# kuldeepbrd1/graspLDM

Measured on AMD Instinct MI355X. Metric: grasps/sec whole-node (1024-pt cloud, 100 DDIM steps), higher is better.
Workload: dtype f32 (GEMMs as split-f16 x3 partial products on the f16 matrix pipe, f32 accumulation; GroupNorm / LayerNorm / attention / scheduler in f32); 1 GPU; LDM mode, 256 synthetic 1024-pt clouds per GPU x 20 grasps, 100 DDIM steps: BASELINE.json configs[2] per GPU (configs[3] = this per-GPU workload on 8 GPUs); experiment=fpc, clouds_per_gpu=256, grasps_per_cloud=20, points=1024, ddim_steps=100, encoder=PVCNNEncoder (shipped fpc config), parallelism=cloud-sharded x1, weights=synthetic recipe seed 0, streams=3

## Files before the change

### graspldm_amd/csrc/quad_narrow.h

```cpp
#ifndef GLDM_QUAD_NARROW_H_
#define GLDM_QUAD_NARROW_H_

#ifdef GLDM_DEBUG_KNOBS
__device__ long long g_q_stamp[4][16];
#define GLDM_QSTAMP(c, i) do { if (blockIdx.x == 0 && (c).lane == 0) g_q_stamp[(c).wave & 3][i] = (long long)__builtin_readcyclecounter(); } while (0)
#else
#define GLDM_QSTAMP(c, i) do {} while (0)
#endif

template <int CTRL>
__device__ __forceinline__ float dpp_zero(float x) {
  return __int_as_float(__builtin_amdgcn_update_dpp(0, __float_as_int(x), CTRL, 0xf, 0xf, true));
}
template <int CTRL>
__device__ __forceinline__ u32x4 dpp_zero4(const u32x4 &v) {
  u32x4 o;
#pragma unroll
  for (int i = 0; i < 4; ++i) o[i] = (unsigned)__builtin_amdgcn_update_dpp(0, (int)v[i], CTRL, 0xf, 0xf, true);
  return o;
}
__device__ __forceinline__ float pos_sum(float v) {
  v += dpp_mov<0x124>(v);
  return v + dpp_mov<0x128>(v);
}
__device__ __forceinline__ float pos_max(float v) { return dpp_max<0x128>(dpp_max<0x124>(v)); }
#define GLDM_DPP8_STAGE1(op, i, j) "v_" op "_f32_dpp %" #i ", %" #j ", %" #j " row_ror:4 row_mask:0xf bank_mask:0xf\n\t"
#define GLDM_DPP8_STAGE2(op, i) "v_" op "_f32_dpp %" #i ", %" #i ", %" #i " row_ror:8 row_mask:0xf bank_mask:0xf\n\t"
#define GLDM_DPP8(op)                                                                                                  \
  "s_nop 1\n\t"                                                                                                         \
  GLDM_DPP8_STAGE1(op, 0, 8) GLDM_DPP8_STAGE1(op, 1, 9) GLDM_DPP8_STAGE1(op, 2, 10) GLDM_DPP8_STAGE1(op, 3, 11)          \
  GLDM_DPP8_STAGE1(op, 4, 12) GLDM_DPP8_STAGE1(op, 5, 13) GLDM_DPP8_STAGE1(op, 6, 14) GLDM_DPP8_STAGE1(op, 7, 15)        \
  GLDM_DPP8_STAGE2(op, 0) GLDM_DPP8_STAGE2(op, 1) GLDM_DPP8_STAGE2(op, 2) GLDM_DPP8_STAGE2(op, 3)                        \
  GLDM_DPP8_STAGE2(op, 4) GLDM_DPP8_STAGE2(op, 5) GLDM_DPP8_STAGE2(op, 6) GLDM_DPP8_STAGE2(op, 7)
#define GLDM_DPP8_OPERANDS                                                                                             \
  : "=&v"(r[0]), "=&v"(r[1]), "=&v"(r[2]), "=&v"(r[3]), "=&v"(r[4]), "=&v"(r[5]), "=&v"(r[6]), "=&v"(r[7])            \
  : "v"(x[0]), "v"(x[1]), "v"(x[2]), "v"(x[3]), "v"(x[4]), "v"(x[5]), "v"(x[6]), "v"(x[7])
#define GLDM_DPP8_STAGE1I(op, i) "v_" op "_f32_dpp %" #i ", %" #i ", %" #i " row_ror:4 row_mask:0xf bank_mask:0xf\n\t"
__device__ __forceinline__ void pos_max8(float (&x)[8]) {
  asm("s_nop 1\n\t"
      GLDM_DPP8_STAGE1I("max", 0) GLDM_DPP8_STAGE1I("max", 1) GLDM_DPP8_STAGE1I("max", 2) GLDM_DPP8_STAGE1I("max", 3)
      GLDM_DPP8_STAGE1I("max", 4) GLDM_DPP8_STAGE1I("max", 5) GLDM_DPP8_STAGE1I("max", 6) GLDM_DPP8_STAGE1I("max", 7)
      GLDM_DPP8_STAGE2("max", 0) GLDM_DPP8_STAGE2("max", 1) GLDM_DPP8_STAGE2("max", 2) GLDM_DPP8_STAGE2("max", 3)
      GLDM_DPP8_STAGE2("max", 4) GLDM_DPP8_STAGE2("max", 5) GLDM_DPP8_STAGE2("max", 6) GLDM_DPP8_STAGE2("max", 7)
      : "+v"(x[0]), "+v"(x[1]), "+v"(x[2]), "+v"(x[3]), "+v"(x[4]), "+v"(x[5]), "+v"(x[6]), "+v"(x[7]));
}
__device__ __forceinline__ void pos_sum8(const float (&x)[8], float (&r)[8]) {
  asm(GLDM_DPP8("add") GLDM_DPP8_OPERANDS);
}
__device__ __forceinline__ float kq_sum(float v) { return half_sum(row_pair_sum(v)); }
__device__ __forceinline__ float kq_max(float v) { return half_max(row_pair_max(v)); }

__device__ __forceinline__ void qsplit8(const f32x4 &a, const f32x4 &b, u32x4 (&pl)[kSplit]) {
  unsigned h, l;
  split_f16x2(a[0], a[1], h, l); pl[0][0] = h; pl[1][0] = l;
  split_f16x2(a[2], a[3], h, l); pl[0][1] = h; pl[1][1] = l;
  split_f16x2(b[0], b[1], h, l); pl[0][2] = h; pl[1][2] = l;
  split_f16x2(b[2], b[3], h, l); pl[0][3] = h; pl[1][3] = l;
}

enum { QM_OUT0 = 0, QM_SS2, QM_C1_2, QM_C2_2, QM_SS3, QM_C1_3, QM_C2_3, QM_QKV1, QM_OUT1, QM_DOWN1,
       QM_SS4, QM_C1_4, QM_C2_4, QM_SS5, QM_C1_5, QM_C2_5, QM_QKV2, QM_OUT2, QM_DOWN2, QM_COUNT };
struct QOff { int mat, a, b; };
constexpr QOff qconv_frag(int mat, int MT, int KB, int i, int mt0 = 0) {
  const int st = i / MT, mi = i % MT, kb = st / 3, t = st % 3;
  const int f = (mt0 + mi) * 3 * KB + t * KB + kb;
  return QOff{mat, 2048 * f, 2048 * f + 1024};
}
constexpr QOff qrb_frag(int mss, int MT, int KB, int i) {
  if (i < MT) return QOff{mss, 1024 * i, 1024 * (MT + i)};
  i -= MT;
  if (i < 3 * KB * MT) return qconv_frag(mss + 1, MT, KB, i);
  return qconv_frag(mss + 2, MT, KB, i - 3 * KB * MT);
}
constexpr int qrb_len(int MT, int KB) { return MT + 6 * KB * MT; }
constexpr QOff qatt_frag(int mqkv, int MT, int KB, int i) {
  const int per = 6 * KB + MT, h = i / per, r = i % per;
  if (r < 6 * KB) {
    const int mt6 = r / KB, kb = r % KB, part = mt6 / 2, half = mt6 % 2;
    const int f = (2 * h + half + 8 * part) * KB + kb;
    return QOff{mqkv, 2048 * f, 2048 * f + 1024};
  }
  const int f = (r - 6 * KB) * 4 + h;
  return QOff{mqkv + 1, 2048 * f, 2048 * f + 1024};
}
constexpr int qatt_len(int MT, int KB) { return 4 * (6 * KB + MT); }
constexpr int qlevel_len(int MT, int KB) { return 2 * qrb_len(MT, KB) + qatt_len(MT, KB) + 2 * MT * 3 * KB; }
constexpr QOff qlevel_frag(int m0, int MT, int KB, int DP, int i) {
  if (i < qrb_len(MT, KB)) return qrb_frag(m0, MT, KB, i);
  i -= qrb_len(MT, KB);
  if (i < qrb_len(MT, KB)) return qrb_frag(m0 + 3, MT, KB, i);
  i -= qrb_len(MT, KB);
  if (i < qatt_len(MT, KB)) return qatt_frag(m0 + 6, MT, KB, i);
  i -= qatt_len(MT, KB);
  const int pass = i / (DP * 3 * KB);
  return qconv_frag(m0 + 8, DP, KB, i % (DP * 3 * KB), DP * pass);
}
constexpr int kQN0 = 0;
constexpr int kQN1 = 4;
constexpr int kQN2 = kQN1 + qlevel_len(2, 1);
constexpr int kQNEnd = kQN2 + qlevel_len(4, 2);
constexpr QOff qstream_off(int n) {
  if (n < kQN1) return QOff{QM_OUT0, 2048 * n, 2048 * n + 1024};
  if (n < kQN2) return qlevel_frag(QM_SS2, 2, 1, 4, n - kQN1);
  return qlevel_frag(QM_SS4, 4, 2, 4, n - kQN2);
}

constexpr int kQG = 4;
constexpr int kQS = 32;
constexpr int kQGroups = kQNEnd / kQG;
static_assert(kQNEnd % kQG == 0 && kQS % kQG == 0, "whole groups");
constexpr int kQR = 6;
constexpr int kQSpinMax = 1 << 20;
__host__ __device__ constexpr int qslot_floats(int s) { return (s < 16 ? PG<4>::kH : PG<4>::kX + 4 * PG<4>::kBlockFloats) + (s & 15) * 512; }
static_assert(PG<4>::kH + 16 * 512 <= PG<4>::kX && PG<4>::kX + 4 * PG<4>::kBlockFloats + 16 * 512 <= 512 * 64, "slot regions");
typedef __attribute__((address_space(3))) int lds_i;
struct QStream4 {
  static constexpr int kEnd = kQNEnd, kGroups = kQGroups;
  static constexpr QOff off(int n) { return qstream_off(n); }
  __host__ __device__ static constexpr int slot_floats(int s) { return qslot_floats(s); }
};

struct QRing {
  u32x4 s[kQR][2];
  float *lds;
  lds_i *sync;
  int lane, quad;
  int flag;
  int spins = 0;
};
__device__ __forceinline__ int lds_poll(const lds_i *p) {
  int v;
  asm volatile("ds_read_b32 %0, %1\n\ts_waitcnt lgkmcnt(0)" : "=v"(v) : "v"(p) : "memory");
  return __builtin_amdgcn_readfirstlane(v);
}
template <int N, class ST = QStream4>
__device__ __forceinline__ void qring_load(QRing &ring) {
  if constexpr (N < ST::kEnd) {
    if constexpr (N % kQG == 0) {
      constexpr int g = N / kQG;
#if defined(GLDM_DEBUG_KNOBS) && defined(GLDM_QEXP_DUP)
      if (false) {
#else
      if (__builtin_expect(ring.flag != g + 1, 0)) {
#endif
        for (int spin = 0; spin < kQSpinMax && lds_poll(ring.sync + (g & 7)) != g + 1; ++spin) {
          __builtin_amdgcn_s_sleep(1);
#ifdef GLDM_DEBUG_KNOBS
          ++ring.spins;
#endif
        }
      }
      if constexpr (g + 1 < ST::kGroups) ring.flag = *(volatile lds_i *)(ring.sync + ((g + 1) & 7));
    }
#if defined(GLDM_DEBUG_KNOBS) && defined(GLDM_QEXP_NOLOAD)
    if (N >= kQR) return;
#endif
    const lds_u4 *slot = (const lds_u4 *)(ring.lds + ST::slot_floats(N % kQS)) + ring.lane;
    ring.s[N % kQR][0] = slot[0];
    ring.s[N % kQR][1] = slot[64];
  }
}
template <int N, class ST = QStream4>
__device__ __forceinline__ f32x4 qring_mfma(QRing &ring, const u32x4 (&b)[kSplit], f32x4 acc) {
#if defined(GLDM_DEBUG_KNOBS) && defined(GLDM_QEXP_NOMFMA)
  acc[0] += __uint_as_float(ring.s[N % kQR][0][0] ^ b[0][0]);
#else
  acc = mfma_split(ring.s[N % kQR], b, acc);
#endif
  if constexpr (N % kQG == kQG - 1) ring.sync[16 + 64 * ring.quad + ring.lane] = N / kQG + 1;
  if constexpr (N >= 1) qring_load<N - 1 + kQR, ST>(ring);
  return acc;
}

typedef __attribute__((address_space(3))) void lds_void;
typedef __attribute__((address_space(1))) const void glob_void;
__device__ __forceinline__ void quad_build_table(const gldm_r1d_desc &d, int *qtab, int tid, int nthreads) {
  const int mbf[QM_COUNT] = {d.lv[0].out_wq,
                             d.rb[2].ss_w, d.rb[2].c1_wq, d.rb[2].c2_wq, d.rb[3].ss_w, d.rb[3].c1_wq, d.rb[3].c2_wq,
                             d.lv[1].qkvn_wq, d.lv[1].out_wq, d.lv[1].down_wq,
                             d.rb[4].ss_w, d.rb[4].c1_wq, d.rb[4].c2_wq, d.rb[5].ss_w, d.rb[5].c1_wq, d.rb[5].c2_wq,
                             d.lv[2].qkvn_wq, d.lv[2].out_wq, d.lv[2].down_wq};
  for (int n = tid; n < kQNEnd; n += nthreads) {
    const QOff o = qstream_off(n);
    int base = 0;
#pragma unroll
    for (int m = 0; m < QM_COUNT; ++m) base = o.mat == m ? mbf[m] * 4 : base;
    qtab[2 * n] = base + o.a;
    qtab[2 * n + 1] = base + o.b;
  }
}
template <class ST = QStream4>
__device__ __forceinline__ void quad_loader(const Ctx &c) {
  using GG = Geo<64>;
  lds_i *sync = (lds_i *)(c.lds + GG::kMiscQ);
  const lds_i *qtab = (const lds_i *)(c.lds + GG::kMiscQTab);
  const char *wb = reinterpret_cast<const char *>(c.w) + c.lane * 16;
  for (int g = c.wave - 4; g < ST::kGroups; g += 4) {
    if (g >= 8) {
      for (int spin = 0; spin < kQSpinMax; ++spin) {
        const int d0 = lds_poll(sync + 16), d1 = lds_poll(sync + 80), d2 = lds_poll(sync + 144), d3 = lds_poll(sync + 208);
        if (min(min(d0, d1), min(d2, d3)) >= g - 7) break;
        __builtin_amdgcn_s_sleep(2);
      }
    }
    const int s0 = (g & 7) * kQG;
#pragma unroll
    for (int f = 0; f < kQG; ++f) {
      const int n = g * kQG + f;
      const int oa = __builtin_amdgcn_readfirstlane(qtab[2 * n]), ob = __builtin_amdgcn_readfirstlane(qtab[2 * n + 1]);
      const int sl = s0 + f;
      float *slot = c.lds + ST::slot_floats(sl);
      __builtin_amdgcn_global_load_lds((glob_void *)(wb + oa), (lds_void *)slot, 16, 0, 0);
      __builtin_amdgcn_global_load_lds((glob_void *)(wb + ob), (lds_void *)(slot + 256), 16, 0, 0);
    }
    asm volatile("s_waitcnt vmcnt(0)" ::: "memory");
    if (c.lane == 0) sync[g & 7] = g + 1;
  }
}

template <int N0, int MT, int KB, int SH = 4, class ST = QStream4>
__device__ __forceinline__ void qconv3(QRing &ring, const u32x4 (&xp)[KB][kSplit], f32x4 (&acc)[MT]) {
  using std::integral_constant;
  auto body = [&](auto st_c) {
    constexpr int st = decltype(st_c)::value, kb = st / 3, t = st % 3;
    u32x4 bs[kSplit];
#pragma unroll
    for (int pl = 0; pl < kSplit; ++pl)
      bs[pl] = t == 1 ? xp[kb][pl] : (t == 0 ? dpp_zero4<0x110 + SH>(xp[kb][pl]) : dpp_zero4<0x100 + SH>(xp[kb][pl]));
    auto per_m = [&](auto mi_c) {
      constexpr int mi = decltype(mi_c)::value;
      acc[mi] = qring_mfma<N0 + st * MT + mi, ST>(ring, bs, acc[mi]);
    };
    per_m(integral_constant<int, 0>{});
    if constexpr (MT > 1) per_m(integral_constant<int, 1>{});
    if constexpr (MT > 2) { per_m(integral_constant<int, 2>{}); per_m(integral_constant<int, 3>{}); }
    __builtin_amdgcn_sched_barrier(0);
  };
  body(integral_constant<int, 0>{}); body(integral_constant<int, 1>{}); body(integral_constant<int, 2>{});
  if constexpr (KB > 1) { body(integral_constant<int, 3>{}); body(integral_constant<int, 4>{}); body(integral_constant<int, 5>{}); }
}

template <int MT, int CPG>
__device__ __forceinline__ void qgn_stats(const f32x4 (&acc)[MT], float (&mean)[MT], float (&var)[MT]) {
  static_assert(CPG == 8 || CPG == 16, "groups of half an m-tile or a whole one");
  constexpr float inv_n = 1.0f / (float)(CPG * 4);
#pragma unroll
  for (int mi = 0; mi < MT; ++mi) {
    float s = (acc[mi][0] + acc[mi][1]) + (acc[mi][2] + acc[mi][3]);
    s = row_pair_sum(pos_sum(s));
    if (CPG == 16) s = half_sum(s);
    const float m = s * inv_n;
    float v = 0.f;
#pragma unroll
    for (int r = 0; r < 4; ++r) {
      const float d = acc[mi][r] - m;
      v = fmaf(d, d, v);
    }
    v = row_pair_sum(pos_sum(v));
    if (CPG == 16) v = half_sum(v);
    mean[mi] = m;
    var[mi] = v * inv_n;
  }
}

struct QRb { int c1_b, n1_w, n1_b, c2_b, n2_w, n2_b, ss_b; };

template <int N0, int MT, int KB>
__device__ __forceinline__ void quad_resblock(const Ctx &c, QRing &ring, const QRb &rb, f32x4 (&xr)[MT],
                                              u32x4 (&xp)[KB][kSplit], int smp) {
  using GG = Geo<64>;
  using std::integral_constant;
  constexpr int C = 16 * MT, CPG = C / 4;
  const int kq = c.lane >> 4;
  const float *w = c.w;
  const lds_f *Gs = (const lds_f *)(c.lds + GG::kMiscG) + smp * 16;
  float gb[4];
#pragma unroll
  for (int j = 0; j < 4; ++j) gb[j] = Gs[4 * j + kq];
  f32x4 sc[MT], sh[MT], g1[MT], be1[MT], b1[MT];
#pragma unroll
  for (int mi = 0; mi < MT; ++mi) {
    const int row0 = 16 * mi + 4 * kq;
    sc[mi] = *reinterpret_cast<const f32x4 *>(w + rb.ss_b + row0);
    sh[mi] = *reinterpret_cast<const f32x4 *>(w + rb.ss_b + C + row0);
    b1[mi] = *reinterpret_cast<const f32x4 *>(w + rb.c1_b + row0);
    g1[mi] = *reinterpret_cast<const f32x4 *>(w + rb.n1_w + row0);
    be1[mi] = *reinterpret_cast<const f32x4 *>(w + rb.n1_b + row0);
  }
  {
    auto ss_m = [&](auto mi_c) {
      constexpr int mi = decltype(mi_c)::value;
      const u32x4 a_sc = ring.s[(N0 + mi) % kQR][0], a_sh = ring.s[(N0 + mi) % kQR][1];
#pragma unroll
      for (int j = 0; j < 4; ++j) {
        sc[mi] = __builtin_amdgcn_mfma_f32_16x16x4f32(__uint_as_float(a_sc[j]), gb[j], sc[mi], 0, 0, 0);
        sh[mi] = __builtin_amdgcn_mfma_f32_16x16x4f32(__uint_as_float(a_sh[j]), gb[j], sh[mi], 0, 0, 0);
      }
      if constexpr (N0 + mi >= 1) qring_load<N0 + mi - 1 + kQR>(ring);
    };
    ss_m(integral_constant<int, 0>{}); ss_m(integral_constant<int, 1>{});
    if constexpr (MT > 2) { ss_m(integral_constant<int, 2>{}); ss_m(integral_constant<int, 3>{}); }
  }
  __builtin_amdgcn_sched_barrier(0);
  f32x4 acc[MT];
#pragma unroll
  for (int mi = 0; mi < MT; ++mi) acc[mi] = f32x4{0.f, 0.f, 0.f, 0.f};
  qconv3<N0 + MT, MT, KB>(ring, xp, acc);
  f32x4 b2[MT], g2[MT], be2[MT];
#pragma unroll
  for (int mi = 0; mi < MT; ++mi) {
    const int row0 = 16 * mi + 4 * kq;
    b2[mi] = *reinterpret_cast<const f32x4 *>(w + rb.c2_b + row0);
    g2[mi] = *reinterpret_cast<const f32x4 *>(w + rb.n2_w + row0);
    be2[mi] = *reinterpret_cast<const f32x4 *>(w + rb.n2_b + row0);
  }
#pragma unroll
  for (int mi = 0; mi < MT; ++mi)
#pragma unroll
    for (int r = 0; r < 4; ++r) acc[mi][r] += b1[mi][r];
  float mean[MT], var[MT];
  qgn_stats<MT, CPG>(acc, mean, var);
  constexpr float kR = sqrt_up(CPG * 4);
  float hb = 0.f;
#pragma unroll
  for (int mi = 0; mi < MT; ++mi)
#pragma unroll
    for (int r = 0; r < 4; ++r)
      hb = fmaxf(hb, fmaf(__builtin_fabsf(g1[mi][r] * sc[mi][r]), kR, __builtin_fabsf(fmaf(be1[mi][r], sc[mi][r], sh[mi][r]))));
  hb = kq_max(pos_max(hb));
  int e = (int)((__float_as_uint(hb) >> 23) & 0xffu) - 127 - 14;
  e = e < 0 ? 0 : e;
  const float hinv = __uint_as_float((unsigned)(127 - e) << 23), hs = __uint_as_float((unsigned)(127 + e) << 23);
  u32x4 hp[KB][kSplit];
#pragma unroll
  for (int mi = 0; mi < MT; ++mi) {
    const float rstd = __builtin_amdgcn_rsqf(var[mi] + 1e-5f);
#pragma unroll
    for (int r = 0; r < 4; ++r) {
      float A = rstd * g1[mi][r];
      float B = be1[mi][r] - mean[mi] * A;
      B = B * sc[mi][r] + sh[mi][r];
      A = A * sc[mi][r];
      acc[mi][r] = silu(fmaf(acc[mi][r], A, B)) * hinv;
    }
  }
#pragma unroll
  for (int kb = 0; kb < KB; ++kb) qsplit8(acc[2 * kb], acc[2 * kb + 1], hp[kb]);
#pragma unroll
  for (int mi = 0; mi < MT; ++mi) acc[mi] = f32x4{0.f, 0.f, 0.f, 0.f};
  qconv3<N0 + MT + 3 * KB * MT, MT, KB>(ring, hp, acc);
#pragma unroll
  for (int mi = 0; mi < MT; ++mi)
#pragma unroll
    for (int r = 0; r < 4; ++r) acc[mi][r] = fmaf(b2[mi][r], hinv, acc[mi][r]);
  qgn_stats<MT, CPG>(acc, mean, var);
#pragma unroll
  for (int mi = 0; mi < MT; ++mi) {
    const float rstd = __builtin_amdgcn_rsqf((var[mi] * hs) * hs + 1e-5f) * hs;
#pragma unroll
    for (int r = 0; r < 4; ++r) {
      const float A = rstd * g2[mi][r];
      xr[mi][r] += silu(fmaf(acc[mi][r], A, be2[mi][r] - mean[mi] * A));
    }
  }
#pragma unroll
  for (int kb = 0; kb < KB; ++kb) qsplit8(xr[2 * kb], xr[2 * kb + 1], xp[kb]);
}

template <int J>
__device__ __forceinline__ float fmac_ror(float acc, float a, float b) {
  static_assert(J >= 1 && J <= 3, "rotations by 4, 8, 12 lanes");
  if constexpr (J == 1) asm("v_fmac_f32_dpp %0, %1, %2 row_ror:4 row_mask:0xf bank_mask:0xf" : "+v"(acc) : "v"(a), "v"(b));
  else if constexpr (J == 2) asm("v_fmac_f32_dpp %0, %1, %2 row_ror:8 row_mask:0xf bank_mask:0xf" : "+v"(acc) : "v"(a), "v"(b));
  else asm("v_fmac_f32_dpp %0, %1, %2 row_ror:12 row_mask:0xf bank_mask:0xf" : "+v"(acc) : "v"(a), "v"(b));
  return acc;
}
template <bool L2E>
__device__ __forceinline__ void quad_attention_head(const f32x4 (&qa)[2], const f32x4 (&ka)[2], const f32x4 (&va)[2], f32x4 (&out)[2]) {
  constexpr float kL2e = 1.44269504088896340736f;
  float kn[2][4], qe[2][4];
  {
    float m8[8], e8[8], s8[8];
#pragma unroll
    for (int i = 0; i < 8; ++i) m8[i] = ka[i >> 2][i & 3];
    pos_max8(m8);
#pragma unroll
    for (int i = 0; i < 8; ++i) {
      const float d = ka[i >> 2][i & 3] - m8[i];
      e8[i] = L2E ? __builtin_amdgcn_exp2f(d) : __builtin_amdgcn_exp2f(d * kL2e);
    }
    pos_sum8(e8, s8);
#pragma unroll
    for (int i = 0; i < 8; ++i) kn[i >> 2][i & 3] = e8[i] * __builtin_amdgcn_rcpf(s8[i]);
  }
  float qm = fmaxf(fmaxf(fmaxf(qa[0][0], qa[0][1]), fmaxf(qa[0][2], qa[0][3])), fmaxf(fmaxf(qa[1][0], qa[1][1]), fmaxf(qa[1][2], qa[1][3])));
  qm = kq_max(qm);
  float qs = 0.f;
#pragma unroll
  for (int h = 0; h < 2; ++h)
#pragma unroll
    for (int r = 0; r < 4; ++r) {
      qe[h][r] = L2E ? __builtin_amdgcn_exp2f(qa[h][r] - qm) : __builtin_amdgcn_exp2f((qa[h][r] - qm) * kL2e);
      qs += qe[h][r];
    }
  const float qscale = 0.17677669529663687f * __builtin_amdgcn_rcpf(kq_sum(qs));
  __builtin_amdgcn_sched_barrier(0);
  asm volatile("s_nop 1");
  float A[4];
  {
    float a0 = 0.f, a1 = 0.f, a2 = 0.f, a3 = 0.f;
#pragma unroll
    for (int h = 0; h < 2; ++h)
#pragma unroll
      for (int r = 0; r < 4; ++r) {
        a0 = fmaf(kn[h][r], qe[h][r], a0);
        a1 = fmac_ror<1>(a1, kn[h][r], qe[h][r]);
        a2 = fmac_ror<2>(a2, kn[h][r], qe[h][r]);
        a3 = fmac_ror<3>(a3, kn[h][r], qe[h][r]);
      }
    A[0] = kq_sum(a0) * qscale; A[1] = kq_sum(a1) * qscale; A[2] = kq_sum(a2) * qscale; A[3] = kq_sum(a3) * qscale;
  }
#pragma unroll
  for (int h = 0; h < 2; ++h)
#pragma unroll
    for (int r = 0; r < 4; ++r) {
      float o = va[h][r] * A[0];
      o = fmac_ror<1>(o, va[h][r], A[1]);
      o = fmac_ror<2>(o, va[h][r], A[2]);
      o = fmac_ror<3>(o, va[h][r], A[3]);
      out[h][r] = o;
    }
}

struct QLv { int qkvn_s, out_b, ln2_g; };

template <int N0, int MT, int KB>
__device__ __forceinline__ void quad_attention(const Ctx &c, QRing &ring, const QLv &lv, f32x4 (&xr)[MT],
                                               u32x4 (&xp)[KB][kSplit]) {
  using std::integral_constant;
  constexpr int C = 16 * MT, kPer = 6 * KB + MT;
  const int kq = c.lane >> 4;
  const float *w = c.w;
  float s = 0.f;
#pragma unroll
  for (int mi = 0; mi < MT; ++mi) s += (xr[mi][0] + xr[mi][1]) + (xr[mi][2] + xr[mi][3]);
  const float mean = kq_sum(s) * (1.0f / (float)C);
  float v = 0.f;
#pragma unroll
  for (int mi = 0; mi < MT; ++mi)
#pragma unroll
    for (int r = 0; r < 4; ++r) {
      const float d = xr[mi][r] - mean;
      v = fmaf(d, d, v);
    }
  const float rstd = __builtin_amdgcn_rsqf(kq_sum(v) * (1.0f / (float)C) + 1e-5f);
  u32x4 xn[KB][kSplit];
  {
    const float mr = mean * rstd;
    f32x4 t[MT];
#pragma unroll
    for (int mi = 0; mi < MT; ++mi)
#pragma unroll
      for (int r = 0; r < 4; ++r) t[mi][r] = fmaf(xr[mi][r], rstd, -mr);
#pragma unroll
    for (int kb = 0; kb < KB; ++kb) qsplit8(t[2 * kb], t[2 * kb + 1], xn[kb]);
  }
  f32x4 oacc[MT];
#pragma unroll
  for (int mi = 0; mi < MT; ++mi) oacc[mi] = *reinterpret_cast<const f32x4 *>(w + lv.out_b + 16 * mi + 4 * kq);
  auto head = [&](auto h_c) {
    constexpr int h = decltype(h_c)::value, NH = N0 + h * kPer;
    f32x4 qkv[6];
#pragma unroll
    for (int i = 0; i < 6; ++i) qkv[i] = f32x4{0.f, 0.f, 0.f, 0.f};
    auto mt6 = [&](auto i_c) {
      constexpr int i = decltype(i_c)::value;
      qkv[i] = qring_mfma<NH + i * KB>(ring, xn[0], qkv[i]);
      if constexpr (KB > 1) qkv[i] = qring_mfma<NH + i * KB + 1>(ring, xn[KB - 1], qkv[i]);
    };
    mt6(integral_constant<int, 0>{}); mt6(integral_constant<int, 1>{}); mt6(integral_constant<int, 2>{});
    mt6(integral_constant<int, 3>{}); mt6(integral_constant<int, 4>{}); mt6(integral_constant<int, 5>{});
    f32x4 o[2];
    const f32x4 qa[2] = {qkv[0], qkv[1]}, ka[2] = {qkv[2], qkv[3]}, va[2] = {qkv[4], qkv[5]};
    quad_attention_head<true>(qa, ka, va, o);
    u32x4 op[kSplit];
    qsplit8(o[0], o[1], op);
    auto om = [&](auto mi_c) {
      constexpr int mi = decltype(mi_c)::value;
      oacc[mi] = qring_mfma<NH + 6 * KB + mi>(ring, op, oacc[mi]);
    };
    om(integral_constant<int, 0>{}); om(integral_constant<int, 1>{});
    if constexpr (MT > 2) { om(integral_constant<int, 2>{}); om(integral_constant<int, 3>{}); }
  };
  head(integral_constant<int, 0>{}); head(integral_constant<int, 1>{}); head(integral_constant<int, 2>{}); head(integral_constant<int, 3>{});
  float s1 = 0.f;
#pragma unroll
  for (int mi = 0; mi < MT; ++mi) s1 += (oacc[mi][0] + oacc[mi][1]) + (oacc[mi][2] + oacc[mi][3]);
  const float m2 = kq_sum(s1) * (1.0f / (float)C);
  float v2 = 0.f;
#pragma unroll
  for (int mi = 0; mi < MT; ++mi)
#pragma unroll
    for (int r = 0; r < 4; ++r) {
      const float d = oacc[mi][r] - m2;
      v2 = fmaf(d, d, v2);
    }
  const float rs2 = __builtin_amdgcn_rsqf(kq_sum(v2) * (1.0f / (float)C) + 1e-5f);
#pragma unroll
  for (int mi = 0; mi < MT; ++mi) {
    const f32x4 gv = *reinterpret_cast<const f32x4 *>(w + lv.ln2_g + 16 * mi + 4 * kq);
#pragma unroll
    for (int r = 0; r < 4; ++r) xr[mi][r] += (oacc[mi][r] - m2) * rs2 * gv[r];
  }
#pragma unroll
  for (int kb = 0; kb < KB; ++kb) qsplit8(xr[2 * kb], xr[2 * kb + 1], xp[kb]);
}

struct QRb4 { int c1_w, c1_b, n1_w, n1_b, c2_w, c2_b, n2_w, n2_b, ss_w, ss_b; };

__device__ __forceinline__ f32x4 q4_weights(const float *w, int off, int lane) {
  const int i = lane & 15, kq = lane >> 4;
  f32x4 f = *reinterpret_cast<const f32x4 *>(w + off + ((kq * 16 + (i >> 2)) * 4));
  if (i & 3) f = f32x4{0.f, 0.f, 0.f, 0.f};
  return f;
}
__device__ __forceinline__ float q4_conv(const f32x4 &wt, float bias, float x) {
  f32x4 acc = f32x4{bias, 0.f, 0.f, 0.f};
  acc = __builtin_amdgcn_mfma_f32_16x16x4f32(wt[0], dpp_zero<0x114>(x), acc, 0, 0, 0);
  acc = __builtin_amdgcn_mfma_f32_16x16x4f32(wt[1], x, acc, 0, 0, 0);
  acc = __builtin_amdgcn_mfma_f32_16x16x4f32(wt[2], dpp_zero<0x104>(x), acc, 0, 0, 0);
  return acc[0];
}
__device__ __forceinline__ float q4_gn(float y, float gamma, float beta) {
  const float m = pos_sum(y) * 0.25f;
  const float d = y - m;
  const float rs = __builtin_amdgcn_rsqf(pos_sum(d * d) * 0.25f + 1e-5f);
  return d * rs * gamma + beta;
}
struct QRb4W { f32x4 w1, w2, wss; float b1, g1, be1, b2, g2, be2, ssb0, ssb1; };
__device__ __forceinline__ QRb4W quad_resblock4_load(const Ctx &c, const QRb4 &rb) {
  const int i = c.lane & 15, kq = c.lane >> 4;
  const float *w = c.w;
  QRb4W p;
  p.w1 = q4_weights(w, rb.c1_w, c.lane);
  p.w2 = q4_weights(w, rb.c2_w, c.lane);
  const int srow = (i & 3) == 0 ? (i >> 2) : 4 + (i >> 2);
  p.wss = *reinterpret_cast<const f32x4 *>(w + rb.ss_w + ((kq * 16 + srow) * 4));
  if ((i & 3) > 1) p.wss = f32x4{0.f, 0.f, 0.f, 0.f};
  p.b1 = w[rb.c1_b + kq]; p.g1 = w[rb.n1_w + kq]; p.be1 = w[rb.n1_b + kq];
  p.b2 = w[rb.c2_b + kq]; p.g2 = w[rb.n2_w + kq]; p.be2 = w[rb.n2_b + kq];
  p.ssb0 = w[rb.ss_b + kq]; p.ssb1 = w[rb.ss_b + 4 + kq];
  return p;
}
__device__ __forceinline__ float quad_resblock4(const Ctx &c, const QRb4W &p, float x, int smp) {
  using GG = Geo<64>;
  const int kq = c.lane >> 4;
  f32x4 ss = f32x4{p.ssb0, p.ssb1, 0.f, 0.f};
  const lds_f *Gs = (const lds_f *)(c.lds + GG::kMiscG) + smp * 16;
#pragma unroll
  for (int j = 0; j < 4; ++j) ss = __builtin_amdgcn_mfma_f32_16x16x4f32(p.wss[j], Gs[4 * j + kq], ss, 0, 0, 0);
  float y = q4_conv(p.w1, p.b1, x);
  y = silu(q4_gn(y, p.g1, p.be1) * ss[0] + ss[1]);
  float z = q4_conv(p.w2, p.b2, y);
  z = silu(q4_gn(z, p.g2, p.be2));
  return x + z;
}

struct QLv4 { int qkvn_w, out_b, ln2_g; };

__device__ __forceinline__ float quad_attention4(const Ctx &c, QRing &ring, const QLv4 &lv, float x) {
  using std::integral_constant;
  const int kq = c.lane >> 4;
  const float *w = c.w;
  float fq[kHeads][6];
#pragma unroll
  for (int h = 0; h < kHeads; ++h)
#pragma unroll
    for (int t = 0; t < 6; ++t)
      fq[h][t] = w[lv.qkvn_w + ((2 * h + (t & 1) + 8 * (t >> 1)) * 64 + c.lane) * 4] * (t < 4 ? 1.44269504088896340736f : 1.0f);
  const float outb = w[lv.out_b + kq], g2 = w[lv.ln2_g + kq];
  const float mean = kq_sum(x) * 0.25f;
  const float d = x - mean;
  const float xn = d * __builtin_amdgcn_rsqf(kq_sum(d * d) * 0.25f + 1e-5f);
  f32x4 oacc = f32x4{outb, 0.f, 0.f, 0.f};
  auto head = [&](auto h_c) {
    constexpr int h = decltype(h_c)::value;
    f32x4 qkv[6];
#pragma unroll
    for (int t = 0; t < 6; ++t) qkv[t] = __builtin_amdgcn_mfma_f32_16x16x4f32(fq[h][t], xn, f32x4{0.f, 0.f, 0.f, 0.f}, 0, 0, 0);
    f32x4 o[2];
    const f32x4 qa[2] = {qkv[0], qkv[1]}, ka[2] = {qkv[2], qkv[3]}, va[2] = {qkv[4], qkv[5]};
    quad_attention_head<true>(qa, ka, va, o);
    u32x4 op[kSplit];
    qsplit8(o[0], o[1], op);
    oacc = qring_mfma<kQN0 + h>(ring, op, oacc);
  };
  head(integral_constant<int, 0>{}); head(integral_constant<int, 1>{}); head(integral_constant<int, 2>{}); head(integral_constant<int, 3>{});
  const float y = oacc[0];
  const float m2 = kq_sum(y) * 0.25f;
  const float d2 = y - m2;
  return x + d2 * __builtin_amdgcn_rsqf(kq_sum(d2 * d2) * 0.25f + 1e-5f) * g2;
}

typedef __attribute__((address_space(4))) const gldm_r1d_desc kernarg_desc;
#define GLDM_QDESC() asm volatile("" : "+s"(dk))
__device__ __forceinline__ void quad_narrow_levels(const Ctx &c, kernarg_desc *dk) {
  using GG = Geo<64>;
  using std::integral_constant;
  const int q = c.wave & 3, col = c.lane & 15, kq = c.lane >> 4;
  const int p = col >> 2, sl = col & 3;
  const int smp = 4 * q + sl;
  const int pmcol = 16 * p + smp;
  const float *w = c.w;
  QRing ring;
  ring.lds = c.lds;
  ring.sync = (lds_i *)(c.lds + GG::kMiscQ);
  ring.lane = c.lane;
  ring.quad = q;
  ring.flag = 0;
  GLDM_QSTAMP(c, 0);
  qring_load<0>(ring); qring_load<1>(ring); qring_load<2>(ring); qring_load<3>(ring); qring_load<4>(ring); qring_load<5>(ring);
  static_assert(kQR == 6, "priming loads");
#define GLDM_QRB4(i) QRb4{dk->rb[i].c1_w, dk->rb[i].c1_b, dk->rb[i].n1_w, dk->rb[i].n1_b, dk->rb[i].c2_w, dk->rb[i].c2_b, dk->rb[i].n2_w, dk->rb[i].n2_b, dk->rb[i].ss_w, dk->rb[i].ss_b}
#define GLDM_QRB(i) QRb{dk->rb[i].c1_b, dk->rb[i].n1_w, dk->rb[i].n1_b, dk->rb[i].c2_b, dk->rb[i].n2_w, dk->rb[i].n2_b, dk->rb[i].ss_b}
#define GLDM_QLV(i) QLv{dk->lv[i].qkvn_s, dk->lv[i].out_b, dk->lv[i].ln2_g}
  GLDM_QDESC();
  const QRb4W p0 = quad_resblock4_load(c, GLDM_QRB4(0)), p1 = quad_resblock4_load(c, GLDM_QRB4(1));
  float x = ((const lds_f *)(c.lds + GG::kBufX))[pswz(kq, pmcol)];
  x = quad_resblock4(c, p0, x, smp);
  GLDM_QSTAMP(c, 1);
  x = quad_resblock4(c, p1, x, smp);
  GLDM_QSTAMP(c, 2);
  GLDM_QDESC();
  x = quad_attention4(c, ring, QLv4{dk->lv[0].qkvn_w, dk->lv[0].out_b, dk->lv[0].ln2_g}, x);
  GLDM_QSTAMP(c, 3);
  f32x4 x32[2];
  u32x4 xp32[1][kSplit];
  {
    GLDM_QDESC();
    const WStream wd(w + dk->lv[0].down_w, c.lane);
    const float xl = dpp_zero<0x114>(x), xrr = dpp_zero<0x104>(x);
#pragma unroll
    for (int mi = 0; mi < 2; ++mi) {
      const f32x4 a = wd[(size_t)mi * 64];
      f32x4 acc = *reinterpret_cast<const f32x4 *>(w + dk->lv[0].down_b + 16 * mi + 4 * kq);
      acc = __builtin_amdgcn_mfma_f32_16x16x4f32(a[0], xl, acc, 0, 0, 0);
      acc = __builtin_amdgcn_mfma_f32_16x16x4f32(a[1], x, acc, 0, 0, 0);
      acc = __builtin_amdgcn_mfma_f32_16x16x4f32(a[2], xrr, acc, 0, 0, 0);
      x32[mi] = acc;
    }
    qsplit8(x32[0], x32[1], xp32[0]);
  }
  GLDM_QSTAMP(c, 4);
  constexpr int kRb1 = qrb_len(2, 1), kAtt1 = qatt_len(2, 1);
  GLDM_QDESC();
  quad_resblock<kQN1, 2, 1>(c, ring, GLDM_QRB(2), x32, xp32, smp);
  GLDM_QSTAMP(c, 5);
  GLDM_QDESC();
  quad_resblock<kQN1 + kRb1, 2, 1>(c, ring, GLDM_QRB(3), x32, xp32, smp);
  GLDM_QSTAMP(c, 6);
  GLDM_QDESC();
  quad_attention<kQN1 + 2 * kRb1, 2, 1>(c, ring, GLDM_QLV(1), x32, xp32);
  GLDM_QSTAMP(c, 7);
  f32x4 x64[4];
  u32x4 xp64[2][kSplit];
  {
    GLDM_QDESC();
    const int down_b1 = dk->lv[1].down_b;
#pragma unroll
    for (int mi = 0; mi < 4; ++mi) x64[mi] = *reinterpret_cast<const f32x4 *>(w + down_b1 + 16 * mi + 4 * kq);
    qconv3<kQN1 + 2 * kRb1 + kAtt1, 4, 1>(ring, xp32, x64);
    qsplit8(x64[0], x64[1], xp64[0]);
    qsplit8(x64[2], x64[3], xp64[1]);
  }
  GLDM_QSTAMP(c, 8);
  constexpr int kRb2 = qrb_len(4, 2), kAtt2 = qatt_len(4, 2);
  GLDM_QDESC();
  quad_resblock<kQN2, 4, 2>(c, ring, GLDM_QRB(4), x64, xp64, smp);
  GLDM_QSTAMP(c, 9);
  GLDM_QDESC();
  quad_resblock<kQN2 + kRb2, 4, 2>(c, ring, GLDM_QRB(5), x64, xp64, smp);
  GLDM_QSTAMP(c, 10);
  GLDM_QDESC();
  quad_attention<kQN2 + 2 * kRb2, 4, 2>(c, ring, GLDM_QLV(2), x64, xp64);
  GLDM_QSTAMP(c, 11);
  {
    lds_f *X3 = (lds_f *)(c.lds + GG::kBufX);
    GLDM_QDESC();
    const int down_b2 = dk->lv[2].down_b;
    auto pass = [&](auto h_c) {
      constexpr int half = decltype(h_c)::value;
      f32x4 acc[4];
#pragma unroll
      for (int mi = 0; mi < 4; ++mi) acc[mi] = *reinterpret_cast<const f32x4 *>(w + down_b2 + 16 * (4 * half + mi) + 4 * kq);
      qconv3<kQN2 + 2 * kRb2 + kAtt2 + 24 * half, 4, 2>(ring, xp64, acc);
#pragma unroll
      for (int mi = 0; mi < 4; ++mi) {
        const int row0 = 16 * (4 * half + mi) + 4 * kq;
#pragma unroll
        for (int r = 0; r < 4; ++r) X3[pswz(row0 + r, pmcol)] = acc[mi][r];
        store_planes4<4>(c.lds + PG<4>::kX, row0, pmcol, acc[mi][0], acc[mi][1], acc[mi][2], acc[mi][3]);
      }
    };
    pass(integral_constant<int, 0>{}); pass(integral_constant<int, 1>{});
  }
  GLDM_QSTAMP(c, 12);
#ifdef GLDM_DEBUG_KNOBS
  if (blockIdx.x == 0 && c.lane == 0) g_q_stamp[c.wave & 3][13] = ring.spins;
#endif
  static_assert(kQN2 + 2 * kRb2 + kAtt2 + 48 == kQNEnd, "stream length");
#undef GLDM_QDESC
#undef GLDM_QRB4
#undef GLDM_QRB
#undef GLDM_QLV
}

#endif
```

Before: 313,700 grasps/s.

## Prefetch per-block weight vectors early to hide global load latency in quad narrow path

Moves small global loads (scale/shift rows, down-conv biases, LN gains, attention4 projection weights) ahead of the compute that uses them. An early hook is added to resblocks and attention so the next stage's vectors are issued during the current stage's MFMA work. The ring priming loads are moved after the level-0 resblocks. The intent is to hide global-memory latency on the critical path, at the cost of higher register pressure from holding more prefetched values live.

```diff
diff --git a/graspldm_amd/csrc/quad_narrow.h b/graspldm_amd/csrc/quad_narrow.h
--- a/graspldm_amd/csrc/quad_narrow.h
+++ b/graspldm_amd/csrc/quad_narrow.h
@@ -264,10 +264,20 @@
 }
 
 struct QRb { int c1_b, n1_w, n1_b, c2_b, n2_w, n2_b, ss_b; };
-
-template <int N0, int MT, int KB>
+template <int MT>
+__device__ __forceinline__ void qrb_ss_rows(const float *w, int ss_b, int kq, f32x4 (&ssb)[2 * MT]) {
+#pragma unroll
+  for (int mi = 0; mi < MT; ++mi) {
+    const int row0 = 16 * mi + 4 * kq;
+    ssb[mi] = *reinterpret_cast<const f32x4 *>(w + ss_b + row0);
+    ssb[MT + mi] = *reinterpret_cast<const f32x4 *>(w + ss_b + 16 * MT + row0);
+  }
+}
+struct QNoHook { __device__ __forceinline__ void operator()() const {} };
+
+template <int N0, int MT, int KB, class F = QNoHook>
 __device__ __forceinline__ void quad_resblock(const Ctx &c, QRing &ring, const QRb &rb, f32x4 (&xr)[MT],
-                                              u32x4 (&xp)[KB][kSplit], int smp) {
+                                              u32x4 (&xp)[KB][kSplit], int smp, const f32x4 (&ssb)[2 * MT], F &&early = F()) {
   using GG = Geo<64>;
   using std::integral_constant;
   constexpr int C = 16 * MT, CPG = C / 4;
@@ -281,8 +291,8 @@
 #pragma unroll
   for (int mi = 0; mi < MT; ++mi) {
     const int row0 = 16 * mi + 4 * kq;
-    sc[mi] = *reinterpret_cast<const f32x4 *>(w + rb.ss_b + row0);
-    sh[mi] = *reinterpret_cast<const f32x4 *>(w + rb.ss_b + C + row0);
+    sc[mi] = ssb[mi];
+    sh[mi] = ssb[MT + mi];
     b1[mi] = *reinterpret_cast<const f32x4 *>(w + rb.c1_b + row0);
     g1[mi] = *reinterpret_cast<const f32x4 *>(w + rb.n1_w + row0);
     be1[mi] = *reinterpret_cast<const f32x4 *>(w + rb.n1_b + row0);
@@ -346,9 +356,11 @@
   }
 #pragma unroll
   for (int kb = 0; kb < KB; ++kb) qsplit8(acc[2 * kb], acc[2 * kb + 1], hp[kb]);
+  if constexpr (MT < 4) early();
 #pragma unroll
   for (int mi = 0; mi < MT; ++mi) acc[mi] = f32x4{0.f, 0.f, 0.f, 0.f};
   qconv3<N0 + MT + 3 * KB * MT, MT, KB>(ring, hp, acc);
+  if constexpr (MT == 4) early();
 #pragma unroll
   for (int mi = 0; mi < MT; ++mi)
 #pragma unroll
@@ -434,9 +446,9 @@
 
 struct QLv { int qkvn_s, out_b, ln2_g; };
 
-template <int N0, int MT, int KB>
+template <int N0, int MT, int KB, class F = QNoHook>
 __device__ __forceinline__ void quad_attention(const Ctx &c, QRing &ring, const QLv &lv, f32x4 (&xr)[MT],
-                                               u32x4 (&xp)[KB][kSplit]) {
+                                               u32x4 (&xp)[KB][kSplit], F &&early = F()) {
   using std::integral_constant;
   constexpr int C = 16 * MT, kPer = 6 * KB + MT;
   const int kq = c.lane >> 4;
@@ -492,7 +504,12 @@
     om(integral_constant<int, 0>{}); om(integral_constant<int, 1>{});
     if constexpr (MT > 2) { om(integral_constant<int, 2>{}); om(integral_constant<int, 3>{}); }
   };
-  head(integral_constant<int, 0>{}); head(integral_constant<int, 1>{}); head(integral_constant<int, 2>{}); head(integral_constant<int, 3>{});
+  head(integral_constant<int, 0>{}); head(integral_constant<int, 1>{}); head(integral_constant<int, 2>{});
+  f32x4 gv[MT];
+#pragma unroll
+  for (int mi = 0; mi < MT; ++mi) gv[mi] = *reinterpret_cast<const f32x4 *>(w + lv.ln2_g + 16 * mi + 4 * kq);
+  early();
+  head(integral_constant<int, 3>{});
   float s1 = 0.f;
 #pragma unroll
   for (int mi = 0; mi < MT; ++mi) s1 += (oacc[mi][0] + oacc[mi][1]) + (oacc[mi][2] + oacc[mi][3]);
@@ -507,11 +524,9 @@
     }
   const float rs2 = __builtin_amdgcn_rsqf(kq_sum(v2) * (1.0f / (float)C) + 1e-5f);
 #pragma unroll
-  for (int mi = 0; mi < MT; ++mi) {
-    const f32x4 gv = *reinterpret_cast<const f32x4 *>(w + lv.ln2_g + 16 * mi + 4 * kq);
-#pragma unroll
-    for (int r = 0; r < 4; ++r) xr[mi][r] += (oacc[mi][r] - m2) * rs2 * gv[r];
-  }
+  for (int mi = 0; mi < MT; ++mi)
+#pragma unroll
+    for (int r = 0; r < 4; ++r) xr[mi][r] += (oacc[mi][r] - m2) * rs2 * gv[mi][r];
 #pragma unroll
   for (int kb = 0; kb < KB; ++kb) qsplit8(xr[2 * kb], xr[2 * kb + 1], xp[kb]);
 }
@@ -568,17 +583,28 @@
 
 struct QLv4 { int qkvn_w, out_b, ln2_g; };
 
-__device__ __forceinline__ float quad_attention4(const Ctx &c, QRing &ring, const QLv4 &lv, float x) {
-  using std::integral_constant;
+struct QAtt4W { float fq[kHeads][6], outb, g2; };
+__device__ __forceinline__ QAtt4W quad_attention4_load(const Ctx &c, const QLv4 &lv) {
   const int kq = c.lane >> 4;
   const float *w = c.w;
+  QAtt4W p;
+#pragma unroll
+  for (int h = 0; h < kHeads; ++h)
+#pragma unroll
+    for (int t = 0; t < 6; ++t) p.fq[h][t] = w[lv.qkvn_w + ((2 * h + (t & 1) + 8 * (t >> 1)) * 64 + c.lane) * 4];
+  p.outb = w[lv.out_b + kq];
+  p.g2 = w[lv.ln2_g + kq];
+  return p;
+}
+__device__ __forceinline__ float quad_attention4(const Ctx &c, QRing &ring, const QAtt4W &p, float x) {
+  using std::integral_constant;
   float fq[kHeads][6];
 #pragma unroll
   for (int h = 0; h < kHeads; ++h)
 #pragma unroll
     for (int t = 0; t < 6; ++t)
-      fq[h][t] = w[lv.qkvn_w + ((2 * h + (t & 1) + 8 * (t >> 1)) * 64 + c.lane) * 4] * (t < 4 ? 1.44269504088896340736f : 1.0f);
-  const float outb = w[lv.out_b + kq], g2 = w[lv.ln2_g + kq];
+      fq[h][t] = p.fq[h][t] * (t < 4 ? 1.44269504088896340736f : 1.0f);
+  const float outb = p.outb, g2 = p.g2;
   const float mean = kq_sum(x) * 0.25f;
   const float d = x - mean;
   const float xn = d * __builtin_amdgcn_rsqf(kq_sum(d * d) * 0.25f + 1e-5f);
@@ -619,31 +645,40 @@
   ring.quad = q;
   ring.flag = 0;
   GLDM_QSTAMP(c, 0);
-  qring_load<0>(ring); qring_load<1>(ring); qring_load<2>(ring); qring_load<3>(ring); qring_load<4>(ring); qring_load<5>(ring);
-  static_assert(kQR == 6, "priming loads");
 #define GLDM_QRB4(i) QRb4{dk->rb[i].c1_w, dk->rb[i].c1_b, dk->rb[i].n1_w, dk->rb[i].n1_b, dk->rb[i].c2_w, dk->rb[i].c2_b, dk->rb[i].n2_w, dk->rb[i].n2_b, dk->rb[i].ss_w, dk->rb[i].ss_b}
 #define GLDM_QRB(i) QRb{dk->rb[i].c1_b, dk->rb[i].n1_w, dk->rb[i].n1_b, dk->rb[i].c2_b, dk->rb[i].n2_w, dk->rb[i].n2_b, dk->rb[i].ss_b}
 #define GLDM_QLV(i) QLv{dk->lv[i].qkvn_s, dk->lv[i].out_b, dk->lv[i].ln2_g}
   GLDM_QDESC();
   const QRb4W p0 = quad_resblock4_load(c, GLDM_QRB4(0)), p1 = quad_resblock4_load(c, GLDM_QRB4(1));
   float x = ((const lds_f *)(c.lds + GG::kBufX))[pswz(kq, pmcol)];
+  GLDM_QDESC();
+  const QAtt4W pa = quad_attention4_load(c, QLv4{dk->lv[0].qkvn_w, dk->lv[0].out_b, dk->lv[0].ln2_g});
+  f32x4 wd4[2], x32[2], ssb32[2][4];
+  {
+    GLDM_QDESC();
+    const WStream wd(w + dk->lv[0].down_w, c.lane);
+#pragma unroll
+    for (int mi = 0; mi < 2; ++mi) {
+      wd4[mi] = wd[(size_t)mi * 64];
+      x32[mi] = *reinterpret_cast<const f32x4 *>(w + dk->lv[0].down_b + 16 * mi + 4 * kq);
+    }
+    qrb_ss_rows<2>(w, dk->rb[2].ss_b, kq, ssb32[0]);
+  }
   x = quad_resblock4(c, p0, x, smp);
   GLDM_QSTAMP(c, 1);
   x = quad_resblock4(c, p1, x, smp);
   GLDM_QSTAMP(c, 2);
-  GLDM_QDESC();
-  x = quad_attention4(c, ring, QLv4{dk->lv[0].qkvn_w, dk->lv[0].out_b, dk->lv[0].ln2_g}, x);
+  qring_load<0>(ring); qring_load<1>(ring); qring_load<2>(ring); qring_load<3>(ring); qring_load<4>(ring); qring_load<5>(ring);
+  static_assert(kQR == 6, "priming loads");
+  x = quad_attention4(c, ring, pa, x);
   GLDM_QSTAMP(c, 3);
-  f32x4 x32[2];
   u32x4 xp32[1][kSplit];
   {
-    GLDM_QDESC();
-    const WStream wd(w + dk->lv[0].down_w, c.lane);
     const float xl = dpp_zero<0x114>(x), xrr = dpp_zero<0x104>(x);
 #pragma unroll
     for (int mi = 0; mi < 2; ++mi) {
-      const f32x4 a = wd[(size_t)mi * 64];
-      f32x4 acc = *reinterpret_cast<const f32x4 *>(w + dk->lv[0].down_b + 16 * mi + 4 * kq);
+      const f32x4 a = wd4[mi];
+      f32x4 acc = x32[mi];
       acc = __builtin_amdgcn_mfma_f32_16x16x4f32(a[0], xl, acc, 0, 0, 0);
       acc = __builtin_amdgcn_mfma_f32_16x16x4f32(a[1], x, acc, 0, 0, 0);
       acc = __builtin_amdgcn_mfma_f32_16x16x4f32(a[2], xrr, acc, 0, 0, 0);
@@ -654,21 +689,27 @@
   GLDM_QSTAMP(c, 4);
   constexpr int kRb1 = qrb_len(2, 1), kAtt1 = qatt_len(2, 1);
   GLDM_QDESC();
-  quad_resblock<kQN1, 2, 1>(c, ring, GLDM_QRB(2), x32, xp32, smp);
+  quad_resblock<kQN1, 2, 1>(c, ring, GLDM_QRB(2), x32, xp32, smp, ssb32[0], [&]() {
+    GLDM_QDESC();
+    qrb_ss_rows<2>(w, dk->rb[3].ss_b, kq, ssb32[1]);
+  });
   GLDM_QSTAMP(c, 5);
+  f32x4 x64[4], ssb64[2][8];
   GLDM_QDESC();
-  quad_resblock<kQN1 + kRb1, 2, 1>(c, ring, GLDM_QRB(3), x32, xp32, smp);
+  quad_resblock<kQN1 + kRb1, 2, 1>(c, ring, GLDM_QRB(3), x32, xp32, smp, ssb32[1]);
   GLDM_QSTAMP(c, 6);
   GLDM_QDESC();
-  quad_attention<kQN1 + 2 * kRb1, 2, 1>(c, ring, GLDM_QLV(1), x32, xp32);
+  quad_attention<kQN1 + 2 * kRb1, 2, 1>(c, ring, GLDM_QLV(1), x32, xp32, [&]() {
+    GLDM_QDESC();
+    const int down_b1 = dk->lv[1].down_b;
+#pragma unroll
+    for (int mi = 0; mi < 4; ++mi) x64[mi] = *reinterpret_cast<const f32x4 *>(w + down_b1 + 16 * mi + 4 * kq);
+  });
   GLDM_QSTAMP(c, 7);
-  f32x4 x64[4];
   u32x4 xp64[2][kSplit];
   {
     GLDM_QDESC();
-    const int down_b1 = dk->lv[1].down_b;
-#pragma unroll
-    for (int mi = 0; mi < 4; ++mi) x64[mi] = *reinterpret_cast<const f32x4 *>(w + down_b1 + 16 * mi + 4 * kq);
+    qrb_ss_rows<4>(w, dk->rb[4].ss_b, kq, ssb64[0]);
     qconv3<kQN1 + 2 * kRb1 + kAtt1, 4, 1>(ring, xp32, x64);
     qsplit8(x64[0], x64[1], xp64[0]);
     qsplit8(x64[2], x64[3], xp64[1]);
@@ -676,23 +717,32 @@
   GLDM_QSTAMP(c, 8);
   constexpr int kRb2 = qrb_len(4, 2), kAtt2 = qatt_len(4, 2);
   GLDM_QDESC();
-  quad_resblock<kQN2, 4, 2>(c, ring, GLDM_QRB(4), x64, xp64, smp);
+  quad_resblock<kQN2, 4, 2>(c, ring, GLDM_QRB(4), x64, xp64, smp, ssb64[0], [&]() {
+    GLDM_QDESC();
+    qrb_ss_rows<4>(w, dk->rb[5].ss_b, kq, ssb64[1]);
+  });
   GLDM_QSTAMP(c, 9);
   GLDM_QDESC();
-  quad_resblock<kQN2 + kRb2, 4, 2>(c, ring, GLDM_QRB(5), x64, xp64, smp);
+  quad_resblock<kQN2 + kRb2, 4, 2>(c, ring, GLDM_QRB(5), x64, xp64, smp, ssb64[1]);
   GLDM_QSTAMP(c, 10);
+  f32x4 db64[2][4];
+  auto down64_rows = [&](int half) {
+    GLDM_QDESC();
+    const int down_b2 = dk->lv[2].down_b;
+#pragma unroll
+    for (int mi = 0; mi < 4; ++mi) db64[half][mi] = *reinterpret_cast<const f32x4 *>(w + down_b2 + 16 * (4 * half + mi) + 4 * kq);
+  };
   GLDM_QDESC();
-  quad_attention<kQN2 + 2 * kRb2, 4, 2>(c, ring, GLDM_QLV(2), x64, xp64);
+  quad_attention<kQN2 + 2 * kRb2, 4, 2>(c, ring, GLDM_QLV(2), x64, xp64, [&]() { down64_rows(0); });
   GLDM_QSTAMP(c, 11);
   {
     lds_f *X3 = (lds_f *)(c.lds + GG::kBufX);
-    GLDM_QDESC();
-    const int down_b2 = dk->lv[2].down_b;
     auto pass = [&](auto h_c) {
       constexpr int half = decltype(h_c)::value;
+      if constexpr (half == 0) down64_rows(1);
       f32x4 acc[4];
 #pragma unroll
-      for (int mi = 0; mi < 4; ++mi) acc[mi] = *reinterpret_cast<const f32x4 *>(w + down_b2 + 16 * (4 * half + mi) + 4 * kq);
+      for (int mi = 0; mi < 4; ++mi) acc[mi] = db64[half][mi];
       qconv3<kQN2 + 2 * kRb2 + kAtt2 + 24 * half, 4, 2>(ring, xp64, acc);
 #pragma unroll
       for (int mi = 0; mi < 4; ++mi) {
```

Result: no change. 316,000 grasps/s (median of 6 runs) (+0.7%).
